# phylo42/EPIK

Hardware: AMD Instinct MI355X
Metric: reads placed/sec (higher is better)
Workload: dtype f32

## Files before the change

### epik_amd/capi.py

```python
from __future__ import annotations

import ctypes
import os

import numpy as np

_HERE = os.path.dirname(os.path.abspath(__file__))
LIB_PATH = os.environ.get("EPIK_AMD_LIB") or os.path.join(_HERE, "libepik_amd.so")

ABI_VERSION = 3

OK, ERR_INVALID, ERR_NO_DEVICE, ERR_HIP, ERR_UNSUPPORTED = 0, 1, 2, 3, 4

PLACEMENT = np.dtype([("branch", np.uint32), ("score", np.float32), ("lwr", np.float64)])
PKDB_VALUE = np.dtype([("branch", np.uint32), ("score", np.float32)])

EXPORTS = (
    "epik_amd_device_count",
    "epik_amd_last_error",
    "epik_amd_placer_create",
    "epik_amd_placer_plan",
    "epik_amd_placer_plan_sizes",
    "epik_amd_placer_build_image",
    "epik_amd_placer_destroy",
    "epik_amd_placer_place",
    "epik_amd_placer_place_device",
    "epik_amd_placer_algorithmic_bytes",
    "epik_amd_placer_create_sharded",
    "epik_amd_placer_accumulate_device",
    "epik_amd_placer_finish_device",
    "epik_amd_placer_partial_info",
    "epik_amd_placer_accumulate_lists_device",
    "epik_amd_placer_finish_lists_device",
    "epik_amd_placer_last_path",
    "epik_amd_placer_stream_build",
    "epik_amd_placer_place_sharded",
    "epik_amd_placer_release_scratch",
    "epik_amd_placer_set_wide_counts",
# ... 154 lines not shown
    lib.epik_amd_placer_release_scratch.restype = i32
    lib.epik_amd_placer_release_scratch.argtypes = [vp]
    lib.epik_amd_placer_stream_build.restype = i32
    lib.epik_amd_placer_stream_build.argtypes = [vp, ctypes.POINTER(ctypes.c_uint32), ctypes.POINTER(ctypes.c_uint32)]
    lib.epik_amd_placer_last_path.restype = i32
    lib.epik_amd_placer_last_path.argtypes = [vp, ctypes.POINTER(ctypes.c_uint32)]
    lib.epik_amd_placer_plan.restype = i32
    lib.epik_amd_placer_plan.argtypes = [ctypes.POINTER(PlacerDesc), ctypes.c_uint32, ctypes.c_uint32, u64,
                                         ctypes.POINTER(Plan)]
    lib.epik_amd_placer_plan_sizes.restype = i32
    lib.epik_amd_placer_plan_sizes.argtypes = [ctypes.c_uint32] * 4 + [ctypes.POINTER(ListBin), u64, ctypes.c_uint32, ctypes.c_uint32,
                                               u64, ctypes.POINTER(Plan)]
    lib.epik_amd_placer_build_image.restype = i32
    lib.epik_amd_placer_build_image.argtypes = [ctypes.POINTER(PlacerDesc), ctypes.c_uint32, ctypes.c_uint32, u64,
                                                vp, vp, vp]
    lib.epik_amd_placer_destroy.restype = None
    lib.epik_amd_placer_destroy.argtypes = [vp]
    lib.epik_amd_placer_place.restype = i32
    lib.epik_amd_placer_place.argtypes = [vp, vp, vp, u64, vp, vp, vp]
    lib.epik_amd_placer_place_device.restype = i32
    lib.epik_amd_placer_place_device.argtypes = [vp, vp, vp, u64, vp, vp, vp, vp]
    lib.epik_amd_placer_algorithmic_bytes.restype = i32
    lib.epik_amd_placer_algorithmic_bytes.argtypes = [vp, vp, vp, u64, vp, vp, ctypes.POINTER(u64)]
    lib.epik_amd_placer_launch_info.restype = i32
    lib.epik_amd_placer_launch_info.argtypes = [vp, ctypes.POINTER(ctypes.c_uint32),
                                                ctypes.POINTER(ctypes.c_uint32),
                                                ctypes.POINTER(ctypes.c_uint32)]
    lib.epik_amd_placer_set_wide_counts.restype = i32
    lib.epik_amd_placer_set_wide_counts.argtypes = [vp, i32]
    lib.epik_amd_placer_choose_counts.restype = i32
# ... 33 lines not shown
```

### epik_amd/csrc/capi.hip

```cpp
#include <hip/hip_runtime.h>

#include <algorithm>
#include <atomic>
#include <cmath>
#include <cstdio>
#include <cstdlib>
#include <cstring>
#include <new>
#include <string>
#include <thread>
#include <vector>

#include "db_image.hpp"
#include "epik_amd.h"
#include "place_kernel.h"
#include "placer_impl.hpp"

namespace {

thread_local std::string g_last_error;

int fail(int code, const std::string &msg)
{
    g_last_error = msg;
// ... 263 lines not shown
    p->device = d->device;
    p->num_keys = d->num_keys;
    p->num_entries = d->num_entries;

    size_t free_mem = 0, total_mem = 0;
    CREATE_TRY(hipMemGetInfo(&free_mem, &total_mem));
    const image::Source src{d, shard_index, shard_count};
    image::Plan &plan = p->plan;
    if (const int rc = image::make_plan(src, free_mem, std::getenv("EPIK_AMD_LAYOUT"), std::getenv("EPIK_AMD_KERNEL"),
                                        plan, err);
        rc != EPIK_AMD_OK) {
        return fail(rc, err);
    }
    p->layout = plan.layout;
    p->team = plan.layout == epik_amd::DbLayout::kTeam;
    p->db_bytes = plan.posting_bytes;
    CREATE_TRY(hipStreamCreateWithFlags(&p->stream, hipStreamNonBlocking));
    CREATE_TRY(hipStreamCreateWithFlags(&p->stream_in, hipStreamNonBlocking));
    CREATE_TRY(hipStreamCreateWithFlags(&p->stream_out, hipStreamNonBlocking));
    CREATE_TRY(hipMalloc(&p->d_table, plan.table_bytes));
    if (plan.filter_bytes) CREATE_TRY(hipMalloc(reinterpret_cast<void **>(&p->d_filter), plan.filter_bytes));
    CREATE_TRY(hipMalloc(reinterpret_cast<void **>(&p->d_postings), plan.posting_bytes));
    {
        DeviceSink table, filter, postings;
        CREATE_TRY(table.init(static_cast<uint8_t *>(p->d_table), plan.table_bytes, p->stream_in));
        if (plan.filter_bytes)
            CREATE_TRY(filter.init(reinterpret_cast<uint8_t *>(p->d_filter), plan.filter_bytes, p->stream_out));
        CREATE_TRY(postings.init(p->d_postings, plan.posting_bytes, p->stream));
        const int rc = image::build(src, plan, table, plan.filter_bytes ? &filter : nullptr, postings, err);
        bool ok_t = true, ok_f = true, ok_p = true;
// ... 114 lines not shown
        for (int counts = 0; counts < 3; ++counts) {
            auto &g = p->geo[counts];
            const uint32_t desc_bytes = epik_amd::kWaveDescBytes;
            g.lds_wave_bytes = epik_amd::wave_lds_bytes(pp.n_pad, counts);
            if (counts == epik_amd::kCounts8 && (pp.n_pad + 7u) / 8u > desc_bytes) {
                g.max_blocks = 0;
                continue;
            }
            if (g.lds_wave_bytes > kMaxLdsPerBlock) {
                return fail(EPIK_AMD_ERR_UNSUPPORTED, "num_branches too large for the one-wavefront-per-read kernel");
            }
            uint32_t best_waves = 0;
            for (uint32_t wpb = 4; wpb >= 1; wpb >>= 1) {
                const uint32_t block_bytes = wpb * g.lds_wave_bytes;
                if (block_bytes > kMaxLdsPerBlock) continue;
                CREATE_TRY(epik_amd::set_place_reads_lds_limit(p->layout, p->plan.runs, counts, block_bytes));
                int per_cu = 0;
                CREATE_TRY(epik_amd::place_reads_occupancy(p->layout, p->plan.runs, counts, (int)(wpb * 64u), block_bytes, &per_cu));
                const uint32_t lds_units = (block_bytes + epik_amd::kLdsGranule - 1u) / epik_amd::kLdsGranule;
                per_cu = std::min<int>(per_cu, (int)(128u / std::max(lds_units, 1u)));
                if (per_cu < 1) per_cu = 1;
                if ((uint32_t)per_cu * wpb > best_waves) {
                    best_waves = (uint32_t)per_cu * wpb;
                    g.waves_per_block = wpb;
                    g.lds_block_bytes = block_bytes;
                    g.max_blocks = (uint32_t)prop.multiProcessorCount * (uint32_t)per_cu;
                }
            }
            g.resident_waves = best_waves;
            CREATE_TRY(epik_amd::set_place_reads_lds_limit(p->layout, p->plan.runs, counts, g.lds_block_bytes));
            CREATE_TRY(epik_amd::set_finish_reads_lds_limit(counts, g.lds_block_bytes));
        }
    }
    if (const char *e = std::getenv("EPIK_AMD_MAX_BLOCKS")) p->max_blocks_cap = (uint32_t)std::strtoul(e, nullptr, 10);
    if (const char *w = std::getenv("EPIK_AMD_WIDE_COUNTS")) {
        p->counts = w[0] == '1' ? epik_amd::kCounts32 : w[0] == '2' ? epik_amd::kCounts8 : epik_amd::kCounts16;
        if (p->counts == epik_amd::kCounts8 && p->geo[epik_amd::kCounts8].max_blocks == 0) p->counts = epik_amd::kCounts16;
        p->counts_forced = true;
    }
#undef CREATE_TRY

    owner.p = nullptr;
    *out = p;
    return EPIK_AMD_OK;
}
// ... 84 lines not shown
    namespace image = epik_amd::image;
    if (!out) return fail(EPIK_AMD_ERR_INVALID, "null argument");
    try {
        std::string err;
        if (const int rc = image::resolve_shard(d, shard_index, shard_count, err); rc != EPIK_AMD_OK) return fail(rc, err);
        if (const int rc = image::validate(d, shard_index, shard_count, err); rc != EPIK_AMD_OK) return fail(rc, err);
        image::Plan plan;
        if (const int rc = image::make_plan(image::Source{d, shard_index, shard_count}, (size_t)free_bytes,
                                            std::getenv("EPIK_AMD_LAYOUT"), std::getenv("EPIK_AMD_KERNEL"), plan, err);
            rc != EPIK_AMD_OK)
            return fail(rc, err);
        fill_plan(plan, out);
        return EPIK_AMD_OK;
    } catch (const std::exception &e) {
        return fail(EPIK_AMD_ERR_INVALID, std::string("plan: ") + e.what());
    }
}

int epik_amd_placer_build_image(const epik_amd_placer_desc *d, uint32_t shard_index, uint32_t shard_count,
                                uint64_t free_bytes, void *table, void *filter, void *postings)
{
    namespace image = epik_amd::image;
    try {
        std::string err;
        if (const int rc = image::resolve_shard(d, shard_index, shard_count, err); rc != EPIK_AMD_OK) return fail(rc, err);
        if (const int rc = image::validate(d, shard_index, shard_count, err); rc != EPIK_AMD_OK) return fail(rc, err);
        image::Plan plan;
        const image::Source src{d, shard_index, shard_count};
        if (const int rc = image::make_plan(src, (size_t)free_bytes, std::getenv("EPIK_AMD_LAYOUT"),
                                            std::getenv("EPIK_AMD_KERNEL"), plan, err);
// ... 243 lines not shown
                tp.read_list = p->d_slow_list;
                tp.read_list_count = p->d_front_cursor + 1;
                HIP_TRY(epik_amd::launch_team(tp, p->team_waves, p->counts, (int)mode, dim3((unsigned)blocks),
                                              g.lds_block_bytes, stream));
                HIP_TRY(hipMemcpyAsync(p->h_front_cursor, p->d_front_cursor, 3 * sizeof(unsigned long long),
                                       hipMemcpyDeviceToHost, stream));
            }
        } else {
            HIP_TRY(epik_amd::launch_team(tp, p->team_waves, p->counts, (int)mode, dim3((unsigned)blocks), g.lds_block_bytes,
                                          stream));
        }
    } else if (mode == kFinish) {
        HIP_TRY(epik_amd::launch_finish_reads(pp, p->counts, dim3((unsigned)blocks), dim3(g.waves_per_block * 64u),
                                              g.lds_block_bytes, stream));
    } else {
        HIP_TRY(epik_amd::launch_place_reads(pp, p->layout, p->plan.runs, p->counts, dim3((unsigned)blocks),
                                             dim3(g.waves_per_block * 64u), g.lds_block_bytes, stream));
    }
    if (timed) {
        HIP_TRY(hipEventRecord(p->ev_stop, stream));
        p->ev_recorded = true;
    }
    return EPIK_AMD_OK;
}

int epik_amd_placer_accumulate_device(epik_amd_placer *p, const void *d_seqs, const void *d_seq_offsets,
                                      uint64_t n, void *d_scores, void *d_counts, const void *d_amb_slot,
                                      void *d_amb_order, void *d_amb_avg, void *stream)
{
    if (!p) return fail(EPIK_AMD_ERR_INVALID, "null placer");
    if (n && (!d_seqs || !d_seq_offsets || !d_scores || !d_counts))
// ... 104 lines not shown
{
    if (!p || !wide || !sparse_quads) return fail(EPIK_AMD_ERR_INVALID, "null argument");
    *wide = *sparse_quads = 0;
    if (!p->team || !p->team_front) return EPIK_AMD_OK;
    const auto &g = p->geo[p->counts];
    const bool is_wide = epik_amd::team_stream_is_wide(p->team_waves, g.stream_lds_bytes[1], g.stream_bw[1]);
    *wide = is_wide ? 1u : 0u;
    *sparse_quads = is_wide && p->counts != epik_amd::kCounts32 ? p->sparse_quads : 0u;
    return EPIK_AMD_OK;
}

int epik_amd_placer_last_path(const epik_amd_placer *p, uint32_t *path)
{
    if (!p || !path) return fail(EPIK_AMD_ERR_INVALID, "null argument");
    *path = !p->team ? EPIK_AMD_PATH_WAVE : p->last_streamed ? EPIK_AMD_PATH_TEAM_STREAMED : EPIK_AMD_PATH_TEAM_ONE_KERNEL;
    return EPIK_AMD_OK;
}

int epik_amd_placer_place_device(epik_amd_placer *p, const void *d_seqs, const void *d_seq_offsets,
                                 uint64_t n, void *d_rows, void *d_n_rows, void *d_kmer_counts,
                                 void *stream)
{
    if (!p) return fail(EPIK_AMD_ERR_INVALID, "null placer");
    if (n && (!d_seqs || !d_seq_offsets || !d_rows || !d_n_rows))
        return fail(EPIK_AMD_ERR_INVALID, "null device buffer");
    HIP_TRY(hipSetDevice(p->device));
    return launch(p, kPlace, d_seqs, d_seq_offsets, n, d_rows, d_n_rows, d_kmer_counts,
                  static_cast<hipStream_t>(stream));
}

// ... 276 lines not shown
```

### epik_amd/csrc/db_image.cpp

```cpp
#include "db_image.hpp"

#include <algorithm>
#include <cmath>
#include <cstdlib>
#include <cstring>
#include <new>
#include <vector>

namespace epik_amd::image {

namespace {

class RecordWriter {
public:
    RecordWriter(Sink &sink, size_t record_bytes, uint64_t total_records)
        : _sink(sink), _record(record_bytes), _left(total_records) {}
    uint8_t *next()
    {
        if (_at == _end) {
            const uint64_t n = std::min<uint64_t>(_left, std::max<size_t>(1, (64u << 10) / _record));
            _at = _sink.reserve((size_t)n * _record);
            _end = _at + (size_t)n * _record;
            _left -= n;
        }
// ... 335 lines not shown

    const WaveLayout w = choose_wave_layout(d->alphabet_size, d->num_keys, plan.present_codes, free_mem, forced_layout);
    const bool paired = w.paired, filtered = w.filtered, packed = w.packed;
    if (!packed) {
        plan.layout = d->offset_bits == 64 ? DbLayout::kCompact64 : DbLayout::kCompact32;
        plan.table_bytes = (d->num_keys + 1) * (d->offset_bits / 8u);
        plan.posting_bytes = plan.kept_entries * 8u + 512u;
        return EPIK_AMD_OK;
    }
    plan.layout = paired ? DbLayout::kPaired : filtered ? DbLayout::kFiltered : DbLayout::kPacked;
    uint64_t lines = 0;
    const uint64_t quarter = d->num_keys / 4;
    if (plan.n_pad > 65536u) return fail(EPIK_AMD_ERR_UNSUPPORTED, "num_branches too large for the packed layouts");
    const uint64_t table_bytes = d->num_keys * (paired ? 16u : 8u) + 8u;
    {
        uint64_t explicit_lines = 0, coded_lines = 0, in_runs = 0;
        Cursor walk(src);
        for (uint64_t key = 0; key < d->num_keys; ++key) {
            uint64_t first = 0;
            const uint64_t len = walk.list(key, &first);
            explicit_lines += (len * 6u + 127u) / 128u;
            const bool run = is_run(d->values + first, len);
            coded_lines += ((run ? len * 4u : len * 6u) + 127u) / 128u;
            if (run) in_runs += len;
        }
        plan.runs = choose_runs(explicit_lines * 128u + table_bytes, coded_lines * 128u + table_bytes, plan.kept_entries, in_runs,
                                plan.wave_resident[kCounts8] >= kWaveKernelWavesPerCu);
    }
    const bool runs = plan.runs;
    Cursor walk(src);
    for (uint64_t key = 0; key < d->num_keys; ++key) {
        if (paired && quarter && key % quarter == 0 && key / quarter < 4) plan.quarter_lines[key / quarter] = lines;
        uint64_t first = 0;
        const uint64_t len = walk.list(key, &first);
        if (len >= 65536u) return fail(EPIK_AMD_ERR_INVALID, "a posting list of 65536 entries or more in a tree of fewer branches");
        lines += run_lines(d->values + first, len, runs);
    }
    if (lines >= (1ull << 32)) return fail(EPIK_AMD_ERR_UNSUPPORTED, "posting region of 512 GiB or more");
    plan.posting_bytes = lines * 128u + 512u;
    size_packed_tables(d->alphabet_size, d->num_keys, w, plan);
// ... 53 lines not shown
        plan.posting_bytes = lines * 128u + 512u;
        posting_bytes_is_bound = true;
        return EPIK_AMD_OK;
    }
    const WaveLayout w = choose_wave_layout(z.alphabet_size, num_keys, plan.present_codes, free_mem, forced_layout);
    if (!w.packed) {
        const uint32_t offset_bits = plan.kept_entries > 0xffffffffull ? 64u : 32u;
        plan.layout = offset_bits == 64 ? DbLayout::kCompact64 : DbLayout::kCompact32;
        plan.table_bytes = (num_keys + 1) * (offset_bits / 8u);
        plan.posting_bytes = plan.kept_entries * 8u + 512u;
        return EPIK_AMD_OK;
    }
    plan.layout = w.paired ? DbLayout::kPaired : w.filtered ? DbLayout::kFiltered : DbLayout::kPacked;
    if (plan.n_pad > 65536u) return fail(EPIK_AMD_ERR_UNSUPPORTED, "num_branches too large for the packed layouts");
    uint64_t explicit_lines = 0, coded_lines = 0;
    for (uint64_t i = 0; i < z.n_bins; ++i) {
        const epik_amd_list_bin &b = z.bins[i];
        if (b.length == 0 || b.lists == 0) continue;
        explicit_lines += b.lists * ((b.length * 6u + 127u) / 128u);
        const uint64_t as_runs = b.length < 65536u ? b.lists_in_runs : 0;
        coded_lines += (b.lists - as_runs) * ((b.length * 6u + 127u) / 128u) + as_runs * ((b.length * 4u + 127u) / 128u);
    }
    const uint64_t packed_table = num_keys * (w.paired ? 16u : 8u) + 8u;
    plan.runs = choose_runs(explicit_lines * 128u + packed_table, coded_lines * 128u + packed_table, plan.kept_entries, in_runs,
                            plan.wave_resident[kCounts8] >= kWaveKernelWavesPerCu);
    uint64_t lines = 0;
    for (uint64_t i = 0; i < z.n_bins; ++i) {
        const epik_amd_list_bin &b = z.bins[i];
        if (b.length == 0 || b.lists == 0) continue;
        if (b.length >= 65536u) return fail(EPIK_AMD_ERR_INVALID, "a posting list of 65536 entries or more in a tree of fewer branches");
        const uint64_t as_runs = plan.runs ? b.lists_in_runs : 0;
        lines += (b.lists - as_runs) * ((b.length * 6u + 127u) / 128u) + as_runs * ((b.length * 4u + 127u) / 128u);
    }
    if (lines >= (1ull << 32)) return fail(EPIK_AMD_ERR_UNSUPPORTED, "posting region of 512 GiB or more");
    plan.posting_bytes = lines * 128u + 512u;
// ... 214 lines not shown
```

### epik_amd/csrc/db_image.hpp

```cpp
#ifndef EPIK_AMD_DB_IMAGE_HPP
#define EPIK_AMD_DB_IMAGE_HPP

#include <cstddef>
#include <cstdint>
#include <string>
#include <vector>

#include "db_layout.h"
#include "epik_amd.h"

namespace epik_amd::image {

struct Source {
    const epik_amd_placer_desc *d = nullptr;
    uint32_t shard_index = 0, shard_count = 1;
    bool sparse() const { return d->keys != nullptr; }
    uint64_t offset_at(uint64_t i) const
    {
        return d->offset_bits == 64 ? static_cast<const uint64_t *>(d->offsets)[i]
                                    : static_cast<const uint32_t *>(d->offsets)[i];
    }
    uint64_t offsets_len() const { return (sparse() ? d->num_present : d->num_keys) + 1; }
    bool kept(uint64_t key) const { return shard_count == 1 || key % shard_count == shard_index; }
};
// ... 41 lines not shown
    uint64_t _pos = 0;
};

struct Plan {
    DbLayout layout = DbLayout::kCompact32;
    uint32_t n_pad = 0;
    int team_waves = 0;
    uint32_t team_passes = 0, team_slice_rows = 0, team_rows_pad = 0;
    uint64_t team_chunks = 0;
    bool team_paired = false;
    std::vector<uint64_t> team_quarter_lines;
    uint64_t table_bytes = 0, filter_bytes = 0, posting_bytes = 0;
    uint32_t filter_rec_bytes = 8;
    uint64_t kept_entries = 0, present_codes = 0;
    bool runs = false;
    uint64_t quarter_lines[4] = {0, 0, 0, 0};
    uint32_t wave_resident[3] = {0, 0, 0};
    uint32_t shard_index = 0, shard_count = 1;
    uint64_t table_keys = 0;
};

inline uint64_t shard_keys(uint64_t num_keys, uint32_t index, uint32_t count)
{
    return count <= 1 ? num_keys : (num_keys > index ? (num_keys - index + count - 1) / count : 0);
}

struct Sink {
    virtual ~Sink() = default;
    virtual uint8_t *reserve(size_t n) = 0;
};

int resolve_shard(const epik_amd_placer_desc *d, uint32_t &shard_index, uint32_t &shard_count, std::string &err);

int validate(const epik_amd_placer_desc *d, uint32_t shard_index, uint32_t shard_count, std::string &err);

// ... 17 lines not shown
```

### epik_amd/csrc/place_device.hpp

```cpp
#ifndef EPIK_AMD_PLACE_DEVICE_HPP
#define EPIK_AMD_PLACE_DEVICE_HPP
#include <hip/hip_runtime.h>
#include <float.h>
#include <stdint.h>

#include <type_traits>

#include "place_kernel.h"

namespace epik_amd {

namespace {

constexpr int kWave = 64;
constexpr int kTilesPerPass = EPIK_AMD_TILES_PER_PASS;
constexpr int kRing = EPIK_AMD_RING;
static_assert((kRing & (kRing - 1)) == 0 && kRing >= 4 && kRing <= 32, "kRing: power of two, one descriptor lane per stage");
constexpr uint32_t kChunkCap = (uint32_t)kTilesPerPass * 64u;

typedef unsigned int v2u __attribute__((ext_vector_type(2)));
typedef unsigned int v4u __attribute__((ext_vector_type(4)));
typedef int v4i __attribute__((ext_vector_type(4)));

__device__ __forceinline__ int lane_id() { return (int)__lane_id(); }
// ... 279 lines not shown
    __device__ static __forceinline__ uint2 load_posting(const PlaceParams &p, uint32_t rows_pad, uint64_t addr,
                                                         uint32_t w, uint32_t j)
    {
        const uint32_t len = length(w);
        if (kRuns && (w >> 16) != 0u)
            return make_uint2(rows_pad - 1u - ((w >> 16) - j), *reinterpret_cast<const uint32_t *>(p.postings + addr + 4ull * j));
        const uint32_t chunk = j >> 6, r = j & 63u;
        const uint32_t rest = len - (chunk << 6);
        const uint32_t cnt = rest < 64u ? rest : 64u;
        const uint8_t *base = p.postings + addr + (uint64_t)chunk * kChunkBytes;
        const uint32_t cell = *reinterpret_cast<const uint16_t *>(base + 4u * cnt + 2u * r);
        return make_uint2(rows_pad - 1u - cell, *reinterpret_cast<const uint32_t *>(base + 4u * r));
    }
};

template <typename Layout>
__device__ __forceinline__ uint64_t chunk_address(const PlaceParams &p, uint64_t addr, uint32_t c)
{
    return (uint64_t)(p.postings + addr + (uint64_t)c * Layout::kChunkBytes);
}
__device__ __forceinline__ uint64_t null_chunk(const PlaceParams &p) { return (uint64_t)p.postings; }

__device__ __forceinline__ uint32_t tile_char(const uint8_t *__restrict__ seq, uint64_t len, uint64_t tile_pos)
{
    const uint64_t pos = tile_pos + (uint64_t)lane_id();
    return seq[pos < len ? pos : len - 1];
}
__device__ __forceinline__ uint32_t tile_class(uint32_t ch, uint64_t len, uint64_t tile_pos,
                                               const uint32_t *__restrict__ char_class)
{
// ... 237 lines not shown
    for (int i = 0; i < kDepth; ++i) {
        if (i == 0 || (uint32_t)i < last_real) {
            uint32_t sa_next = 0, ca_next = 0;
            stage(
                sa, ca, ring_s[i],
                [&]() {
                    if (i + 1 < kDepth) addresses(ring_c[i + 1], std::integral_constant<int, 0>{}, sa_next, ca_next, score_top, count_top);
                },
                []() {});
            sa = sa_next, ca = ca_next;
        }
    }
    if constexpr (!std::is_same_v<std::remove_cvref_t<Cells>, NoCells>) {
#pragma unroll
        for (int i = 0; i < kDepth; ++i) asm volatile("v_mov_b32 %0, %1" : "=v"(cells_out[i]) : "v"(ring_c[i]));
    }
}

struct WaveCtx {
    static constexpr bool kTeam = false;
    static constexpr uint32_t kCandCap = kChunkCap;
    __device__ __forceinline__ bool untouched() const { return false; }
    template <typename Params>
    __device__ __forceinline__ uint32_t rows_pad(const Params &p) const { return p.n_pad; }
    template <typename Params>
    __device__ __forceinline__ uint32_t rows(const Params &p) const { return p.num_branches; }
    __device__ __forceinline__ uint32_t branch_base() const { return 0u; }
    __device__ __forceinline__ uint32_t kmer_size(const PlaceParams &p) const { return p.kmer_size; }
    __device__ __forceinline__ float log_threshold(const PlaceParams &p) const { return p.log_threshold; }
    __device__ __forceinline__ uint32_t keep_at_most(const PlaceParams &p) const { return p.keep_at_most; }
// ... 583 lines not shown
```

### epik_amd/csrc/place_kernel.h

```cpp
#ifndef EPIK_AMD_PLACE_KERNEL_H
#define EPIK_AMD_PLACE_KERNEL_H

#include <hip/hip_runtime.h>
#include <stdint.h>

#include "epik_amd.h"

#include "db_layout.h"

namespace epik_amd {

struct PlaceParams {
    const void *table;
    const uint64_t *filter;
    uint32_t sigma_pow_km1;
    uint32_t filter_rec_bytes;
    const uint8_t *postings;
    const uint32_t *char_class;
    const uint8_t *seqs;
    const uint64_t *seq_offsets;
    uint64_t n_reads;
    epik_amd_placement *rows;
    uint32_t *n_rows;
    uint32_t *kmer_counts;
// ... 76 lines not shown
hipError_t set_team_lds_limit(int waves, int counts, size_t lds_bytes);
hipError_t team_occupancy(int waves, int counts, size_t lds_bytes, int *blocks_per_cu);
hipError_t launch_team_front(const TeamParams &tp, int waves, int counts, bool lists, dim3 grid, hipStream_t stream);
hipError_t launch_team_stream(const TeamParams &tp, int waves, int counts, int mode, int bw, dim3 grid, size_t lds_bytes,
                              hipStream_t stream, const SparseSources *sources = nullptr);
uint64_t sparse_scan_tiles(uint64_t part_reads, uint32_t slices);
hipError_t launch_team_sparse_scan(const TeamParams &tp, int waves, unsigned long long *tile_sums, hipStream_t stream);
hipError_t launch_team_headers(const TeamParams &tp, int waves, int counts, hipStream_t stream);
hipError_t launch_team_merge(const TeamParams &tp, int waves, dim3 grid, hipStream_t stream);
constexpr size_t kTeamPartialBytes = 24;
hipError_t set_team_stream_lds_limit(int waves, int counts, int mode, int bw, size_t lds_bytes);
bool team_stream_is_wide(int waves, size_t lds_bytes, int bw);
hipError_t team_stream_occupancy(int waves, int counts, int mode, int bw, size_t lds_bytes, int *blocks_per_cu);
hipError_t launch_team_algorithmic_bytes(const TeamParams &tp, int waves, unsigned long long *d_total, hipStream_t stream);

hipError_t launch_place_reads(const PlaceParams &p, DbLayout layout, bool runs, int counts, dim3 grid, dim3 block,
                              size_t lds_bytes, hipStream_t stream);
hipError_t set_place_reads_lds_limit(DbLayout layout, bool runs, int counts, size_t lds_bytes);
hipError_t place_reads_occupancy(DbLayout layout, bool runs, int counts, int block_threads, size_t lds_bytes,
                                 int *blocks_per_cu);
hipError_t launch_finish_reads(const PlaceParams &p, int counts, dim3 grid, dim3 block, size_t lds_bytes,
                               hipStream_t stream);
hipError_t set_finish_reads_lds_limit(int counts, size_t lds_bytes);
hipError_t launch_algorithmic_bytes(const PlaceParams &p, DbLayout layout, bool runs, unsigned long long *d_total,
                                    hipStream_t stream);

}
#endif
```

### epik_amd/csrc/place_kernel.hip

```cpp
#include <hip/hip_runtime.h>
#include <stdint.h>

#include <type_traits>

#include "place_device.hpp"

namespace epik_amd {

template <typename Layout, typename CountT>
__global__ __launch_bounds__(256, 5) void place_reads_kernel(PlaceParams p)
{
    extern __shared__ __align__(16) unsigned char lds_raw[];
    const int lane = lane_id();
    const uint32_t wave_in_block = __builtin_amdgcn_readfirstlane(threadIdx.x >> 6);
    const uint32_t waves_per_block = blockDim.x >> 6;

    WaveLds<CountT> lds;
    {
        unsigned char *base = lds_raw + (size_t)wave_in_block * p.lds_wave_bytes;
        lds.carve(base, p.n_pad);
    }
    const uint32_t score_top = __builtin_amdgcn_readfirstlane((uint32_t)(uintptr_t)lds.score + (p.n_pad - 1u) * 4u);
    const uint32_t count_top = __builtin_amdgcn_readfirstlane((uint32_t)(uintptr_t)lds.count +
                                                              (p.n_pad - 1u) * (uint32_t)sizeof(CountT));
// ... 76 lines not shown
            }
            EPIK_STAMP(0)
            uint32_t nch[kTilesPerPass], first[kTilesPerPass];
            uint32_t total = 0;
            bool found_any[kTilesPerPass];
#pragma unroll
            for (int t = 0; t < kTilesPerPass; ++t) {
                nch[t] = (Layout::length(llen[t]) + (uint32_t)kWave - 1u) >> 6;
                found_any[t] = __ballot(nch[t] != 0) != 0;
                first[t] = total;
                if (found_any[t]) {
                    const uint32_t incl = wave_incl_scan_u32(nch[t]);
                    first[t] = total + incl - nch[t];
                    total += __builtin_amdgcn_readlane(incl, 63);
                }
            }
#ifdef EPIK_AMD_ABLATION
            if (p.ablate & 8u) total = 0;
#endif
            auto *chunks = lds.desc;
            EPIK_STAMP(1)
            for (uint32_t w0 = 0; w0 < total; w0 += kChunkCap) {
                const uint32_t n_round = min(total - w0, kChunkCap);
                const uint32_t n_padded = (n_round + (uint32_t)kRing - 1u) & ~((uint32_t)kRing - 1u);
                constexpr uint32_t kOwnChunks = 3;
#pragma unroll
                for (int t = 0; t < kTilesPerPass; ++t) {
                    if (!found_any[t]) continue;
#pragma unroll
                    for (uint32_t c = 0; c < kOwnChunks; ++c) {
// ... 12 lines not shown
                        const uint32_t l_w = __builtin_amdgcn_readlane(llen[t], m);
                        const uint32_t l_len = Layout::length(l_w);
                        const uint64_t l_start = readlane_u64(start[t], m);
                        for (uint32_t c = (uint32_t)lane + kOwnChunks; (c << 6) < l_len; c += kWave) {
                            const uint32_t idx = l_first + c - w0;
                            if (idx < kChunkCap) {
                                const uint32_t rest = l_len - (c << 6);
                                const uint64_t cnt = rest < (uint32_t)kWave ? rest : (uint32_t)kWave;
                                chunks[idx] = Layout::descriptor(p, l_start, l_w, c, cnt);
                            }
                        }
                    }
                }
                if ((uint32_t)lane < n_padded - n_round) chunks[n_round + lane] = Layout::null_descriptor(p);

                stream_round<Layout, CountT, kRing, false>(p, chunks, n_padded, score_top, count_top, nullptr, n_round);
            }
        }

        EPIK_STAMP(2)
        if (any_amb) {
            const int64_t amb_slot = (p.partial_scores && p.amb_slot) ? (int64_t)p.amb_slot[read] : -1;
            place_ambiguous<Layout, CountT>(kp, lds, seq, len, n_kmers, amb_slot, WaveCtx{});
        }

#ifdef EPIK_AMD_ABLATION
        if (p.ablate & 2u) {
            if (lane == 0) p.n_rows[read] = 0;
            if (!(p.ablate & 4u))
                for (uint32_t i = lane; i < p.n_pad; i += kWave) lds.store(i, 0u, 0u);
            continue;
        }
#endif
// ... 69 lines not shown
    });
}

namespace {

template <typename Layout, typename F>
hipError_t dispatch_counts(int counts, F &&f)
{
    switch (counts) {
        case kCounts8: return f.template operator()<Layout, uint8_t>();
        case kCounts16: return f.template operator()<Layout, uint16_t>();
        case kCounts32: return f.template operator()<Layout, uint32_t>();
    }
    return hipErrorInvalidValue;
}
template <typename F>
hipError_t dispatch(DbLayout layout, bool runs, int counts, F &&f)
{
    switch (layout) {
        case DbLayout::kCompact32: return dispatch_counts<CompactLayout<uint32_t>>(counts, f);
        case DbLayout::kCompact64: return dispatch_counts<CompactLayout<uint64_t>>(counts, f);
        case DbLayout::kPacked:
            return runs ? dispatch_counts<PackedLayout<kPlainTable, true>>(counts, f) : dispatch_counts<PackedLayout<kPlainTable>>(counts, f);
        case DbLayout::kPaired:
            return runs ? dispatch_counts<PackedLayout<kPairedTable, true>>(counts, f) : dispatch_counts<PackedLayout<kPairedTable>>(counts, f);
        case DbLayout::kFiltered:
            return runs ? dispatch_counts<PackedLayout<kFilteredTable, true>>(counts, f) : dispatch_counts<PackedLayout<kFilteredTable>>(counts, f);
        case DbLayout::kTeam: break;
    }
    return hipErrorInvalidValue;
}

}

hipError_t launch_place_reads(const PlaceParams &p, DbLayout layout, bool runs, int counts, dim3 grid, dim3 block,
                              size_t lds_bytes, hipStream_t stream)
{
    return dispatch(layout, runs, counts, [&]<typename L, typename C>() {
        hipLaunchKernelGGL((place_reads_kernel<L, C>), grid, block, lds_bytes, stream, p);
        return hipGetLastError();
    });
}

hipError_t set_place_reads_lds_limit(DbLayout layout, bool runs, int counts, size_t )
{
    return dispatch(layout, runs, counts, [&]<typename L, typename C>() {
        return hipFuncSetAttribute(reinterpret_cast<const void *>(&place_reads_kernel<L, C>),
                                   hipFuncAttributeMaxDynamicSharedMemorySize, (int)kLdsPerCu);
    });
}

hipError_t place_reads_occupancy(DbLayout layout, bool runs, int counts, int block_threads, size_t lds_bytes,
                                 int *blocks_per_cu)
{
    return dispatch(layout, runs, counts, [&]<typename L, typename C>() {
        return hipOccupancyMaxActiveBlocksPerMultiprocessor(blocks_per_cu, place_reads_kernel<L, C>,
                                                            block_threads, lds_bytes);
    });
}

hipError_t launch_finish_reads(const PlaceParams &p, int counts, dim3 grid, dim3 block, size_t lds_bytes,
                               hipStream_t stream)
{
    return dispatch_counts<PackedLayout<kPlainTable>>(counts, [&]<typename L, typename C>() {
        hipLaunchKernelGGL((finish_reads_kernel<C>), grid, block, lds_bytes, stream, p);
        return hipGetLastError();
    });
}

hipError_t set_finish_reads_lds_limit(int counts, size_t )
{
    return dispatch_counts<PackedLayout<kPlainTable>>(counts, [&]<typename L, typename C>() {
        return hipFuncSetAttribute(reinterpret_cast<const void *>(&finish_reads_kernel<C>),
                                   hipFuncAttributeMaxDynamicSharedMemorySize, (int)kLdsPerCu);
    });
}

hipError_t launch_algorithmic_bytes(const PlaceParams &p, DbLayout layout, bool runs, unsigned long long *d_total,
                                    hipStream_t stream)
{
    const dim3 block(256);
    const dim3 grid((unsigned)((p.n_reads + 255) / 256));
    return dispatch(layout, runs, kCounts16, [&]<typename L, typename C>() {
        hipLaunchKernelGGL((algorithmic_bytes_kernel<L>), grid, block, 0, stream, p, d_total);
        return hipGetLastError();
    });
}

}
```

### epik_amd/csrc/placer_impl.hpp

```cpp
#ifndef EPIK_AMD_PLACER_IMPL_HPP
#define EPIK_AMD_PLACER_IMPL_HPP
#include <hip/hip_runtime.h>

#include <string>
#include <vector>

#include "db_image.hpp"
#include "epik_amd.h"
#include "place_kernel.h"

struct epik_amd_placer {
    int device = 0;
    epik_amd::DbLayout layout = epik_amd::DbLayout::kCompact32;
    int counts = epik_amd::kCounts16;
    bool counts_forced = false;
    bool timing = false;
    void *d_table = nullptr;
    uint64_t *d_filter = nullptr;
    uint8_t *d_postings = nullptr;
    uint64_t db_bytes = 0;
    uint32_t *d_char_class = nullptr;
    uint64_t generation = 0;
    void *shard_state = nullptr;
    void (*shard_state_free)(void *) = nullptr;
    std::vector<uint32_t> h_char_class;
    epik_amd::PlaceParams params{};
    epik_amd::image::Plan plan{};
    bool team = false;
    int team_waves = 0;
    const uint8_t *team_table = nullptr;
    uint32_t team_passes = 0, team_slice_rows = 0, team_rows_pad = 0;
    bool team_front = false;
    uint8_t *d_front_hdr = nullptr;
    size_t front_hdr_bytes = 0;
    uint8_t *d_finish_hdr = nullptr;
    size_t finish_hdr_bytes = 0;
    uint64_t *d_slow_list = nullptr;
    size_t slow_list_reads = 0;
    void *d_slice_rows = nullptr, *d_slice_sums = nullptr;
    size_t slice_out_reads = 0;
    uint64_t *d_front_pool = nullptr;
    uint64_t front_pool_cap = 0;
// ... 48 lines not shown
```

### include/epik_amd.h

```cpp
#ifndef EPIK_AMD_H
#define EPIK_AMD_H

#include <stddef.h>
#include <stdint.h>

#ifdef __cplusplus
extern "C" {
#endif

#define EPIK_AMD_ABI_VERSION 3

enum epik_amd_status {
    EPIK_AMD_OK = 0,
    EPIK_AMD_ERR_INVALID = 1,
    EPIK_AMD_ERR_NO_DEVICE = 2,
    EPIK_AMD_ERR_HIP = 3,
    EPIK_AMD_ERR_UNSUPPORTED = 4
};

typedef struct {
    uint32_t branch;
    float score;
} epik_amd_pkdb_value;

// ... 44 lines not shown
    uint64_t posting_bytes;
    uint64_t kept_entries;
    uint32_t run_coded;
    uint32_t posting_bytes_is_bound;
} epik_amd_plan;
int epik_amd_placer_plan(const epik_amd_placer_desc *desc, uint32_t shard_index, uint32_t shard_count,
                         uint64_t free_bytes, epik_amd_plan *plan);
typedef struct {
    uint64_t length;
    uint64_t lists;
    uint64_t lists_in_runs;
} epik_amd_list_bin;
int epik_amd_placer_plan_sizes(uint32_t kmer_size, uint32_t alphabet_size, uint32_t num_branches, uint32_t keep_at_most,
                               const epik_amd_list_bin *bins, uint64_t n_bins, uint32_t shard_index, uint32_t shard_count,
                               uint64_t free_bytes, epik_amd_plan *plan);
int epik_amd_placer_build_image(const epik_amd_placer_desc *desc, uint32_t shard_index, uint32_t shard_count,
                                uint64_t free_bytes, void *table, void *filter, void *postings);

void epik_amd_placer_destroy(epik_amd_placer *p);

int epik_amd_placer_place(epik_amd_placer *p, const char *seqs, const uint64_t *seq_offsets,
                          uint64_t n, epik_amd_placement *rows, uint32_t *n_rows,
                          uint32_t *kmer_counts);

int epik_amd_placer_place_device(epik_amd_placer *p, const void *d_seqs, const void *d_seq_offsets,
                                 uint64_t n, void *d_rows, void *d_n_rows, void *d_kmer_counts,
                                 void *stream);

int epik_amd_placer_algorithmic_bytes(epik_amd_placer *p, const void *d_seqs,
                                      const void *d_seq_offsets, uint64_t n, const void *d_n_rows,
// ... 86 lines not shown
```

Baseline: 177.1 million.

## Count run-coded posting lists with LDS difference array instead of per-chunk counts

When every posting list in the database is run-coded, the wave kernel now records each list's branch range as a +1/-1 pair in an LDS difference array. A prefix scan at the end of each read turns that array into per-branch k-mer counts. The streaming loop then carries only score adds, dropping the per-chunk count loads and updates. This adds LDS atomics per list and a scan over all branches per read. It is enabled by default for the packed and paired layouts with 16- or 32-bit counts, and can be forced on or off with an environment variable.

New measurement: 202.1 million, median of 6. +14.1%, better.

```diff
diff --git a/epik_amd/capi.py b/epik_amd/capi.py
--- a/epik_amd/capi.py
+++ b/epik_amd/capi.py
@@ -22,6 +22,8 @@
     "epik_amd_placer_plan",
     "epik_amd_placer_plan_sizes",
     "epik_amd_placer_build_image",
+    "epik_amd_placer_plan_run_counts",
+    "epik_amd_placer_run_counts",
     "epik_amd_placer_destroy",
     "epik_amd_placer_place",
     "epik_amd_placer_place_device",
@@ -206,6 +208,11 @@
     lib.epik_amd_placer_build_image.restype = i32
     lib.epik_amd_placer_build_image.argtypes = [ctypes.POINTER(PlacerDesc), ctypes.c_uint32, ctypes.c_uint32, u64,
                                                 vp, vp, vp]
+    lib.epik_amd_placer_plan_run_counts.restype = i32
+    lib.epik_amd_placer_plan_run_counts.argtypes = [ctypes.POINTER(PlacerDesc), ctypes.c_uint32, ctypes.c_uint32, u64,
+                                                    ctypes.c_uint32, ctypes.POINTER(ctypes.c_uint32)]
+    lib.epik_amd_placer_run_counts.restype = i32
+    lib.epik_amd_placer_run_counts.argtypes = [vp, ctypes.c_uint32, ctypes.POINTER(ctypes.c_uint32)]
     lib.epik_amd_placer_destroy.restype = None
     lib.epik_amd_placer_destroy.argtypes = [vp]
     lib.epik_amd_placer_place.restype = i32
diff --git a/epik_amd/csrc/capi.hip b/epik_amd/csrc/capi.hip
--- a/epik_amd/csrc/capi.hip
+++ b/epik_amd/csrc/capi.hip
@@ -301,6 +301,8 @@
     }
     p->layout = plan.layout;
     p->team = plan.layout == epik_amd::DbLayout::kTeam;
+    const bool run_lists = image::run_counts_apply(plan, std::getenv("EPIK_AMD_RUN_COUNTS"));
+    p->runs = run_lists ? epik_amd::kRunLists : plan.runs ? epik_amd::kRunsMixed : 0;
     p->db_bytes = plan.posting_bytes;
     CREATE_TRY(hipStreamCreateWithFlags(&p->stream, hipStreamNonBlocking));
     CREATE_TRY(hipStreamCreateWithFlags(&p->stream_in, hipStreamNonBlocking));
@@ -445,9 +447,9 @@
             for (uint32_t wpb = 4; wpb >= 1; wpb >>= 1) {
                 const uint32_t block_bytes = wpb * g.lds_wave_bytes;
                 if (block_bytes > kMaxLdsPerBlock) continue;
-                CREATE_TRY(epik_amd::set_place_reads_lds_limit(p->layout, p->plan.runs, counts, block_bytes));
+                CREATE_TRY(epik_amd::set_place_reads_lds_limit(p->layout, p->runs, counts, block_bytes));
                 int per_cu = 0;
-                CREATE_TRY(epik_amd::place_reads_occupancy(p->layout, p->plan.runs, counts, (int)(wpb * 64u), block_bytes, &per_cu));
+                CREATE_TRY(epik_amd::place_reads_occupancy(p->layout, p->runs, counts, (int)(wpb * 64u), block_bytes, &per_cu));
                 const uint32_t lds_units = (block_bytes + epik_amd::kLdsGranule - 1u) / epik_amd::kLdsGranule;
                 per_cu = std::min<int>(per_cu, (int)(128u / std::max(lds_units, 1u)));
                 if (per_cu < 1) per_cu = 1;
@@ -459,7 +461,7 @@
                 }
             }
             g.resident_waves = best_waves;
-            CREATE_TRY(epik_amd::set_place_reads_lds_limit(p->layout, p->plan.runs, counts, g.lds_block_bytes));
+            CREATE_TRY(epik_amd::set_place_reads_lds_limit(p->layout, p->runs, counts, g.lds_block_bytes));
             CREATE_TRY(epik_amd::set_finish_reads_lds_limit(counts, g.lds_block_bytes));
         }
     }
@@ -574,6 +576,29 @@
         return EPIK_AMD_OK;
     } catch (const std::exception &e) {
         return fail(EPIK_AMD_ERR_INVALID, std::string("plan: ") + e.what());
+    }
+}
+
+int epik_amd_placer_plan_run_counts(const epik_amd_placer_desc *d, uint32_t shard_index, uint32_t shard_count,
+                                    uint64_t free_bytes, uint32_t counts, uint32_t *lists)
+{
+    namespace image = epik_amd::image;
+    if (!lists) return fail(EPIK_AMD_ERR_INVALID, "null argument");
+    if (counts > (uint32_t)epik_amd::kCounts32) return fail(EPIK_AMD_ERR_INVALID, "counts must be 0, 1 or 2");
+    try {
+        std::string err;
+        if (const int rc = image::resolve_shard(d, shard_index, shard_count, err); rc != EPIK_AMD_OK) return fail(rc, err);
+        if (const int rc = image::validate(d, shard_index, shard_count, err); rc != EPIK_AMD_OK) return fail(rc, err);
+        image::Plan plan;
+        if (const int rc = image::make_plan(image::Source{d, shard_index, shard_count}, (size_t)free_bytes,
+                                            std::getenv("EPIK_AMD_LAYOUT"), std::getenv("EPIK_AMD_KERNEL"), plan, err);
+            rc != EPIK_AMD_OK)
+            return fail(rc, err);
+        *lists = counts != (uint32_t)epik_amd::kCounts8 &&
+                 image::run_counts_apply(plan, std::getenv("EPIK_AMD_RUN_COUNTS"));
+        return EPIK_AMD_OK;
+    } catch (const std::exception &e) {
+        return fail(EPIK_AMD_ERR_INVALID, std::string("plan_run_counts: ") + e.what());
     }
 }
 
@@ -847,7 +872,7 @@
         HIP_TRY(epik_amd::launch_finish_reads(pp, p->counts, dim3((unsigned)blocks), dim3(g.waves_per_block * 64u),
                                               g.lds_block_bytes, stream));
     } else {
-        HIP_TRY(epik_amd::launch_place_reads(pp, p->layout, p->plan.runs, p->counts, dim3((unsigned)blocks),
+        HIP_TRY(epik_amd::launch_place_reads(pp, p->layout, p->runs, p->counts, dim3((unsigned)blocks),
                                              dim3(g.waves_per_block * 64u), g.lds_block_bytes, stream));
     }
     if (timed) {
@@ -982,6 +1007,14 @@
 {
     if (!p || !path) return fail(EPIK_AMD_ERR_INVALID, "null argument");
     *path = !p->team ? EPIK_AMD_PATH_WAVE : p->last_streamed ? EPIK_AMD_PATH_TEAM_STREAMED : EPIK_AMD_PATH_TEAM_ONE_KERNEL;
+    return EPIK_AMD_OK;
+}
+
+int epik_amd_placer_run_counts(const epik_amd_placer *p, uint32_t counts, uint32_t *lists)
+{
+    if (!p || !lists) return fail(EPIK_AMD_ERR_INVALID, "null argument");
+    if (counts > (uint32_t)epik_amd::kCounts32) return fail(EPIK_AMD_ERR_INVALID, "counts must be 0, 1 or 2");
+    *lists = !p->team && p->runs == epik_amd::kRunLists && counts != (uint32_t)epik_amd::kCounts8;
     return EPIK_AMD_OK;
 }
 
diff --git a/epik_amd/csrc/db_image.cpp b/epik_amd/csrc/db_image.cpp
--- a/epik_amd/csrc/db_image.cpp
+++ b/epik_amd/csrc/db_image.cpp
@@ -373,7 +373,7 @@
     if (plan.n_pad > 65536u) return fail(EPIK_AMD_ERR_UNSUPPORTED, "num_branches too large for the packed layouts");
     const uint64_t table_bytes = d->num_keys * (paired ? 16u : 8u) + 8u;
     {
-        uint64_t explicit_lines = 0, coded_lines = 0, in_runs = 0;
+        uint64_t explicit_lines = 0, coded_lines = 0, in_runs = 0, not_runs = 0;
         Cursor walk(src);
         for (uint64_t key = 0; key < d->num_keys; ++key) {
             uint64_t first = 0;
@@ -382,7 +382,9 @@
             const bool run = is_run(d->values + first, len);
             coded_lines += ((run ? len * 4u : len * 6u) + 127u) / 128u;
             if (run) in_runs += len;
-        }
+            not_runs += len != 0 && !run;
+        }
+        plan.run_lists = not_runs == 0;
         plan.runs = choose_runs(explicit_lines * 128u + table_bytes, coded_lines * 128u + table_bytes, plan.kept_entries, in_runs,
                                 plan.wave_resident[kCounts8] >= kWaveKernelWavesPerCu);
     }
@@ -466,11 +468,13 @@
     plan.layout = w.paired ? DbLayout::kPaired : w.filtered ? DbLayout::kFiltered : DbLayout::kPacked;
     if (plan.n_pad > 65536u) return fail(EPIK_AMD_ERR_UNSUPPORTED, "num_branches too large for the packed layouts");
     uint64_t explicit_lines = 0, coded_lines = 0;
+    plan.run_lists = true;
     for (uint64_t i = 0; i < z.n_bins; ++i) {
         const epik_amd_list_bin &b = z.bins[i];
         if (b.length == 0 || b.lists == 0) continue;
         explicit_lines += b.lists * ((b.length * 6u + 127u) / 128u);
         const uint64_t as_runs = b.length < 65536u ? b.lists_in_runs : 0;
+        if (as_runs != b.lists) plan.run_lists = false;
         coded_lines += (b.lists - as_runs) * ((b.length * 6u + 127u) / 128u) + as_runs * ((b.length * 4u + 127u) / 128u);
     }
     const uint64_t packed_table = num_keys * (w.paired ? 16u : 8u) + 8u;
diff --git a/epik_amd/csrc/db_image.hpp b/epik_amd/csrc/db_image.hpp
--- a/epik_amd/csrc/db_image.hpp
+++ b/epik_amd/csrc/db_image.hpp
@@ -79,11 +79,20 @@
     uint32_t filter_rec_bytes = 8;
     uint64_t kept_entries = 0, present_codes = 0;
     bool runs = false;
+    bool run_lists = false;
     uint64_t quarter_lines[4] = {0, 0, 0, 0};
     uint32_t wave_resident[3] = {0, 0, 0};
     uint32_t shard_index = 0, shard_count = 1;
     uint64_t table_keys = 0;
 };
+
+inline bool run_counts_apply(const Plan &plan, const char *forced)
+{
+    if (!plan.runs || !plan.run_lists || plan.layout == DbLayout::kTeam) return false;
+    if (forced && forced[0] == 'r') return false;
+    if (forced && forced[0] == 'l') return true;
+    return plan.layout != DbLayout::kFiltered;
+}
 
 inline uint64_t shard_keys(uint64_t num_keys, uint32_t index, uint32_t count)
 {
diff --git a/epik_amd/csrc/place_device.hpp b/epik_amd/csrc/place_device.hpp
--- a/epik_amd/csrc/place_device.hpp
+++ b/epik_amd/csrc/place_device.hpp
@@ -317,6 +317,45 @@
     }
 };
 
+template <int kTable>
+struct RunListLayout : PackedLayout<kTable, true> {
+    static constexpr bool kListCounts = true;
+    static constexpr int kWaitLoads = 1;
+    static constexpr int kFields = 2;
+    __device__ static __forceinline__ uint64_t descriptor(const PlaceParams &p, uint64_t addr, uint32_t w, uint32_t c, uint64_t cnt)
+    {
+        const uint32_t line = (uint32_t)(addr >> 7) + 2u * c;
+        const uint32_t row = p.n_pad - 1u - (w >> 16) + (c << 6);
+        return (uint64_t)line | ((uint64_t)((uint32_t)cnt | (row << 7)) << 32);
+    }
+    __device__ static __forceinline__ uint64_t null_descriptor(const PlaceParams &) { return 0ull; }
+    __device__ static __forceinline__ void prepare(const PlaceParams &, uint64_t d, uint32_t (&f)[kFields])
+    {
+        f[0] = (uint32_t)d;
+        f[1] = (uint32_t)(d >> 32);
+    }
+    template <bool kSettled = false>
+    __device__ static __forceinline__ void issue(const PlaceParams &p, const uint32_t (&f)[kFields], uint32_t lane4,
+                                                 uint32_t score_row0, uint32_t score_top, uint32_t &addr, uint32_t &score)
+    {
+        const uint64_t a = (uint64_t)p.postings + ((uint64_t)f[0] << 7);
+        const uint32_t cnt = f[1] & 127u;
+        const uint32_t base = score_row0 + ((f[1] >> 7) << 2);
+        const v4i srd = {(int)(uint32_t)a, (int)((uint32_t)(a >> 32) & 0xffffu), (int)(cnt * 4u), kRawBufferFormat};
+        asm volatile(".if %6 == 0\n\ts_nop 4\n\t.endif\n\t"
+                     "buffer_load_dword %0, %2, %3, 0 offen\n\t"
+                     "v_add_u32 %1, %4, %2\n\t"
+                     "v_min_u32 %1, %5, %1"
+                     : "=&v"(score), "=&v"(addr)
+                     : "v"(lane4), "s"(srd), "s"(base), "s"(score_top), "n"(kSettled ? 1 : 0)
+                     : "memory");
+    }
+};
+template <typename Layout, typename = void>
+struct ListCounts : std::false_type {};
+template <typename Layout>
+struct ListCounts<Layout, std::void_t<decltype(Layout::kListCounts)>> : std::bool_constant<Layout::kListCounts> {};
+
 template <typename Layout>
 __device__ __forceinline__ uint64_t chunk_address(const PlaceParams &p, uint64_t addr, uint32_t c)
 {
@@ -584,6 +623,122 @@
     if constexpr (!std::is_same_v<std::remove_cvref_t<Cells>, NoCells>) {
 #pragma unroll
         for (int i = 0; i < kDepth; ++i) asm volatile("v_mov_b32 %0, %1" : "=v"(cells_out[i]) : "v"(ring_c[i]));
+    }
+}
+
+template <typename Layout, int kDepth = kRing>
+__device__ __forceinline__ void stream_round_lists(const PlaceParams &p, const typename WaveLds<uint32_t>::u64_t *chunks,
+                                                   uint32_t n_padded, uint32_t score_top, uint32_t n_real)
+{
+    typedef __attribute__((address_space(3))) float lds_f32;
+    const int lane = lane_id();
+    const uint32_t lane4 = (uint32_t)lane * 4u;
+    const uint32_t score_row0 = __builtin_amdgcn_readfirstlane(score_top - (p.n_pad - 1u) * 4u);
+    uint32_t ring_a[kDepth], ring_s[kDepth];
+    auto stage = [&](int i, auto wait_count, auto &&meanwhile, auto &&refill) {
+        lds_f32 *cell = (lds_f32 *)(uintptr_t)ring_a[i];
+        const float old_score = *cell;
+        meanwhile();
+        asm volatile("s_waitcnt vmcnt(%0)" ::"n"(decltype(wait_count)::value) : "memory");
+        __builtin_amdgcn_sched_barrier(0);
+        float new_score;
+        asm volatile("v_add_f32 %0, %1, %2" : "=v"(new_score) : "v"(old_score), "v"(ring_s[i]) : "memory");
+        *cell = new_score;
+        refill();
+    };
+    if (n_padded == 0) return;
+    uint64_t d_next = chunks[lane & (kDepth - 1)];
+    {
+        uint32_t field[Layout::kFields];
+        Layout::prepare(p, d_next, field);
+        d_next = chunks[kDepth + (lane & (kDepth - 1))];
+#pragma unroll
+        for (int i = 0; i < kDepth; ++i) {
+            uint32_t f[Layout::kFields];
+#pragma unroll
+            for (int q = 0; q < Layout::kFields; ++q) f[q] = __builtin_amdgcn_readlane(field[q], i);
+            Layout::issue(p, f, lane4, score_row0, score_top, ring_a[i], ring_s[i]);
+        }
+    }
+    for (uint32_t c0 = (uint32_t)kDepth; c0 < n_padded; c0 += kDepth) {
+        uint32_t field[Layout::kFields];
+        Layout::prepare(p, d_next, field);
+        d_next = chunks[c0 + kDepth + (lane & (kDepth - 1))];
+#pragma unroll
+        for (int i = 0; i < kDepth; ++i) {
+            uint32_t f[Layout::kFields];
+            stage(
+                i, std::integral_constant<int, kDepth - 1>{},
+                [&]() {
+#pragma unroll
+                    for (int q = 0; q < Layout::kFields; ++q)
+                        asm volatile("v_readlane_b32 %0, %1, %2" : "=s"(f[q]) : "v"(field[q]), "i"(i));
+                },
+                [&]() { Layout::template issue<true>(p, f, lane4, score_row0, score_top, ring_a[i], ring_s[i]); });
+        }
+    }
+    const uint32_t last_real = n_real ? n_real - (n_padded - (uint32_t)kDepth) : (uint32_t)kDepth;
+#pragma unroll
+    for (int i = 0; i < kDepth; ++i)
+        if (i == 0 || (uint32_t)i < last_real) stage(i, std::integral_constant<int, 0>{}, []() {}, []() {});
+}
+
+template <typename CountT>
+__device__ __forceinline__ void add_run_count(WaveLds<CountT> lds, uint32_t n_pad, uint32_t w)
+{
+    static_assert(sizeof(CountT) != 1, "8-bit counts keep the per-chunk count ring");
+    typedef __attribute__((address_space(3))) uint32_t lds_u32;
+    const uint32_t r0 = n_pad - 1u - (w >> 16), r1 = r0 + (w & 0xffffu);
+    if constexpr (sizeof(CountT) == 2) {
+        lds_u32 *words = (lds_u32 *)lds.count;
+        __atomic_fetch_add(words + (r0 >> 1), 1u << ((r0 & 1u) << 4), __ATOMIC_RELAXED);
+        __atomic_fetch_sub(words + (r1 >> 1), 1u << ((r1 & 1u) << 4), __ATOMIC_RELAXED);
+    } else {
+        __atomic_fetch_add((lds_u32 *)lds.count + r0, 1u, __ATOMIC_RELAXED);
+        __atomic_fetch_sub((lds_u32 *)lds.count + r1, 1u, __ATOMIC_RELAXED);
+    }
+}
+template <typename CountT>
+__device__ __forceinline__ void materialize_counts(WaveLds<CountT> lds, uint32_t n_pad)
+{
+    static_assert(sizeof(CountT) != 1, "8-bit counts keep the per-chunk count ring");
+    typedef __attribute__((address_space(3))) v4u lds_u32x4;
+    constexpr uint32_t kRows = 16, kWords = kRows * (uint32_t)sizeof(CountT) / 4u, kVecs = kWords / 4u;
+    const uint32_t lane = (uint32_t)lane_id();
+    uint32_t carry = 0;
+    for (uint32_t b0 = 0; b0 < n_pad; b0 += kRows * (uint32_t)kWave) {
+        const uint32_t r0 = b0 + lane * kRows;
+        const bool mine = r0 < n_pad;
+        lds_u32x4 *at = (lds_u32x4 *)(lds.count + (mine ? r0 : 0u));
+        uint32_t v[kWords];
+#pragma unroll
+        for (uint32_t q = 0; q < kVecs; ++q) {
+            const v4u x = mine ? at[q] : v4u{0u, 0u, 0u, 0u};
+            v[4 * q] = x.x, v[4 * q + 1] = x.y, v[4 * q + 2] = x.z, v[4 * q + 3] = x.w;
+        }
+        int32_t s = 0;
+#pragma unroll
+        for (uint32_t q = 0; q < kWords; ++q) {
+            if constexpr (sizeof(CountT) == 2) {
+                const int32_t lo = (int32_t)(v[q] << 16) >> 16;
+                const int32_t hi = (int32_t)(v[q] - (uint32_t)lo) >> 16;
+                const int32_t c_lo = s + lo;
+                s = c_lo + hi;
+                v[q] = ((uint32_t)s << 16) + (uint32_t)c_lo;
+            } else {
+                s += (int32_t)v[q];
+                v[q] = (uint32_t)s;
+            }
+        }
+        const uint32_t incl = wave_incl_scan_u32((uint32_t)s);
+        const uint32_t front = carry + incl - (uint32_t)s;
+        const uint32_t add = sizeof(CountT) == 2 ? front * 0x10001u : front;
+        if (mine) {
+#pragma unroll
+            for (uint32_t q = 0; q < kVecs; ++q)
+                at[q] = v4u{v[4 * q] + add, v[4 * q + 1] + add, v[4 * q + 2] + add, v[4 * q + 3] + add};
+        }
+        carry += __builtin_amdgcn_readlane(incl, 63);
     }
 }
 
diff --git a/epik_amd/csrc/place_kernel.h b/epik_amd/csrc/place_kernel.h
--- a/epik_amd/csrc/place_kernel.h
+++ b/epik_amd/csrc/place_kernel.h
@@ -114,15 +114,16 @@
 hipError_t team_stream_occupancy(int waves, int counts, int mode, int bw, size_t lds_bytes, int *blocks_per_cu);
 hipError_t launch_team_algorithmic_bytes(const TeamParams &tp, int waves, unsigned long long *d_total, hipStream_t stream);
 
-hipError_t launch_place_reads(const PlaceParams &p, DbLayout layout, bool runs, int counts, dim3 grid, dim3 block,
+enum : int { kRunsMixed = 1, kRunLists = 2 };
+hipError_t launch_place_reads(const PlaceParams &p, DbLayout layout, int runs, int counts, dim3 grid, dim3 block,
                               size_t lds_bytes, hipStream_t stream);
-hipError_t set_place_reads_lds_limit(DbLayout layout, bool runs, int counts, size_t lds_bytes);
-hipError_t place_reads_occupancy(DbLayout layout, bool runs, int counts, int block_threads, size_t lds_bytes,
+hipError_t set_place_reads_lds_limit(DbLayout layout, int runs, int counts, size_t lds_bytes);
+hipError_t place_reads_occupancy(DbLayout layout, int runs, int counts, int block_threads, size_t lds_bytes,
                                  int *blocks_per_cu);
 hipError_t launch_finish_reads(const PlaceParams &p, int counts, dim3 grid, dim3 block, size_t lds_bytes,
                                hipStream_t stream);
 hipError_t set_finish_reads_lds_limit(int counts, size_t lds_bytes);
-hipError_t launch_algorithmic_bytes(const PlaceParams &p, DbLayout layout, bool runs, unsigned long long *d_total,
+hipError_t launch_algorithmic_bytes(const PlaceParams &p, DbLayout layout, int runs, unsigned long long *d_total,
                                     hipStream_t stream);
 
 }
diff --git a/epik_amd/csrc/place_kernel.hip b/epik_amd/csrc/place_kernel.hip
--- a/epik_amd/csrc/place_kernel.hip
+++ b/epik_amd/csrc/place_kernel.hip
@@ -114,6 +114,11 @@
                     first[t] = total + incl - nch[t];
                     total += __builtin_amdgcn_readlane(incl, 63);
                 }
+            }
+            if constexpr (ListCounts<Layout>::value) {
+#pragma unroll
+                for (int t = 0; t < kTilesPerPass; ++t)
+                    if (found_any[t] && llen[t] != 0u) add_run_count(lds, p.n_pad, llen[t]);
             }
 #ifdef EPIK_AMD_ABLATION
             if (p.ablate & 8u) total = 0;
@@ -156,9 +161,13 @@
                 }
                 if ((uint32_t)lane < n_padded - n_round) chunks[n_round + lane] = Layout::null_descriptor(p);
 
-                stream_round<Layout, CountT, kRing, false>(p, chunks, n_padded, score_top, count_top, nullptr, n_round);
-            }
-        }
+                if constexpr (ListCounts<Layout>::value)
+                    stream_round_lists<Layout, kRing>(p, chunks, n_padded, score_top, n_round);
+                else
+                    stream_round<Layout, CountT, kRing, false>(p, chunks, n_padded, score_top, count_top, nullptr, n_round);
+            }
+        }
+        if constexpr (ListCounts<Layout>::value) materialize_counts(lds, p.n_pad);
 
         EPIK_STAMP(2)
         if (any_amb) {
@@ -258,18 +267,22 @@
     }
     return hipErrorInvalidValue;
 }
+template <int kTable, typename F>
+hipError_t dispatch_runs(int runs, int counts, F &&f)
+{
+    if (runs == kRunLists && counts == kCounts16) return f.template operator()<RunListLayout<kTable>, uint16_t>();
+    if (runs == kRunLists && counts == kCounts32) return f.template operator()<RunListLayout<kTable>, uint32_t>();
+    return runs ? dispatch_counts<PackedLayout<kTable, true>>(counts, f) : dispatch_counts<PackedLayout<kTable>>(counts, f);
+}
 template <typename F>
-hipError_t dispatch(DbLayout layout, bool runs, int counts, F &&f)
+hipError_t dispatch(DbLayout layout, int runs, int counts, F &&f)
 {
     switch (layout) {
         case DbLayout::kCompact32: return dispatch_counts<CompactLayout<uint32_t>>(counts, f);
         case DbLayout::kCompact64: return dispatch_counts<CompactLayout<uint64_t>>(counts, f);
-        case DbLayout::kPacked:
-            return runs ? dispatch_counts<PackedLayout<kPlainTable, true>>(counts, f) : dispatch_counts<PackedLayout<kPlainTable>>(counts, f);
-        case DbLayout::kPaired:
-            return runs ? dispatch_counts<PackedLayout<kPairedTable, true>>(counts, f) : dispatch_counts<PackedLayout<kPairedTable>>(counts, f);
-        case DbLayout::kFiltered:
-            return runs ? dispatch_counts<PackedLayout<kFilteredTable, true>>(counts, f) : dispatch_counts<PackedLayout<kFilteredTable>>(counts, f);
+        case DbLayout::kPacked: return dispatch_runs<kPlainTable>(runs, counts, f);
+        case DbLayout::kPaired: return dispatch_runs<kPairedTable>(runs, counts, f);
+        case DbLayout::kFiltered: return dispatch_runs<kFilteredTable>(runs, counts, f);
         case DbLayout::kTeam: break;
     }
     return hipErrorInvalidValue;
@@ -277,7 +290,7 @@
 
 }
 
-hipError_t launch_place_reads(const PlaceParams &p, DbLayout layout, bool runs, int counts, dim3 grid, dim3 block,
+hipError_t launch_place_reads(const PlaceParams &p, DbLayout layout, int runs, int counts, dim3 grid, dim3 block,
                               size_t lds_bytes, hipStream_t stream)
 {
     return dispatch(layout, runs, counts, [&]<typename L, typename C>() {
@@ -286,7 +299,7 @@
     });
 }
 
-hipError_t set_place_reads_lds_limit(DbLayout layout, bool runs, int counts, size_t )
+hipError_t set_place_reads_lds_limit(DbLayout layout, int runs, int counts, size_t )
 {
     return dispatch(layout, runs, counts, [&]<typename L, typename C>() {
         return hipFuncSetAttribute(reinterpret_cast<const void *>(&place_reads_kernel<L, C>),
@@ -294,7 +307,7 @@
     });
 }
 
-hipError_t place_reads_occupancy(DbLayout layout, bool runs, int counts, int block_threads, size_t lds_bytes,
+hipError_t place_reads_occupancy(DbLayout layout, int runs, int counts, int block_threads, size_t lds_bytes,
                                  int *blocks_per_cu)
 {
     return dispatch(layout, runs, counts, [&]<typename L, typename C>() {
@@ -320,7 +333,7 @@
     });
 }
 
-hipError_t launch_algorithmic_bytes(const PlaceParams &p, DbLayout layout, bool runs, unsigned long long *d_total,
+hipError_t launch_algorithmic_bytes(const PlaceParams &p, DbLayout layout, int runs, unsigned long long *d_total,
                                     hipStream_t stream)
 {
     const dim3 block(256);
diff --git a/epik_amd/csrc/placer_impl.hpp b/epik_amd/csrc/placer_impl.hpp
--- a/epik_amd/csrc/placer_impl.hpp
+++ b/epik_amd/csrc/placer_impl.hpp
@@ -26,6 +26,7 @@
     std::vector<uint32_t> h_char_class;
     epik_amd::PlaceParams params{};
     epik_amd::image::Plan plan{};
+    int runs = 0;
     bool team = false;
     int team_waves = 0;
     const uint8_t *team_table = nullptr;
diff --git a/include/epik_amd.h b/include/epik_amd.h
--- a/include/epik_amd.h
+++ b/include/epik_amd.h
@@ -82,6 +82,9 @@
 int epik_amd_placer_plan_sizes(uint32_t kmer_size, uint32_t alphabet_size, uint32_t num_branches, uint32_t keep_at_most,
                                const epik_amd_list_bin *bins, uint64_t n_bins, uint32_t shard_index, uint32_t shard_count,
                                uint64_t free_bytes, epik_amd_plan *plan);
+int epik_amd_placer_plan_run_counts(const epik_amd_placer_desc *desc, uint32_t shard_index, uint32_t shard_count,
+                                    uint64_t free_bytes, uint32_t counts, uint32_t *lists);
+int epik_amd_placer_run_counts(const epik_amd_placer *p, uint32_t counts, uint32_t *lists);
 int epik_amd_placer_build_image(const epik_amd_placer_desc *desc, uint32_t shard_index, uint32_t shard_count,
                                 uint64_t free_bytes, void *table, void *filter, void *postings);
 
```
